# JuliaParallel/DistributedArrays.jl

Hardware: NVIDIA H100
Metric: GB/s for map! and sum on Float32 DArray (higher is better)
Workload: dtype f32

## Files before the change

### distributedarrays.jl_b200/_broadcast.py

```python
from __future__ import annotations

import ctypes as C
import struct
from typing import Callable, List, Optional, Sequence, Tuple

import numpy as np

from builtins import any as builtins_any

from . import _lib
from ._darray import B200Array, DArray, dab_dtype, darray, makelocal
from .layout import shape_of
from .runtime import runtime

_RANK = {"bool": 0, "i32": 1, "i64": 2, "i128": 3, "f32": 4, "f64": 5}


class _TagTypes(dict):

    def __missing__(self, tag):
        raise _lib.UnsupportedError(_lib.ERR_UNSUPPORTED, f"values of type {tag} have no array element type on the GPU backend "
                                    "(Int128 is served as the value type of mapreduce(f, op, d) only)")


# ... 407 lines not shown
        self.arr, self.scalar, self.tag, self.temp = arr, scalar, tag, temp


def run_local(rt, expr: Expr, out: B200Array, largs: List[LocalArg]):
    n = out.size
    if n == 0:
        return
    out_tag = tag_of(out.dtype)
    full = [a for a in largs if a.arr is not None]
    same = all(a.arr.shape == out.shape or a.arr.size == n and _squeeze(a.arr.shape) == _squeeze(out.shape) for a in full)
    ctx = rt.ctx
    code = dab_dtype(out.dtype)
    rt.last_kernel = "fixed"
    if same and expr.jt == out_tag and out_tag != "bool":
        x0 = largs[0] if largs and largs[0].arr is not None and largs[0].tag == out_tag else None
        if x0 is not None and all(_only_arg0(expr)):
            ab = match_affine(expr)
            if ab is not None:
                a = np.asarray(ab[0], dtype=out.dtype)
                b = np.asarray(ab[1], dtype=out.dtype)
                _lib.call("dab_affine", ctx, code, C.c_void_p(out.ptr), C.c_void_p(x0.arr.ptr), C.c_void_p(a.ctypes.data),
                          C.c_void_p(b.ctypes.data), n)
                rt.last_kernel = "dab_affine"
                return
            if expr.op in _UN and _is_arg(expr.args[0], 0):
                _lib.call("dab_unary", ctx, code, _UN[expr.op], C.c_void_p(out.ptr), C.c_void_p(x0.arr.ptr), n)
                return
            if _is_arg(expr, 0):
                _lib.call("dab_unary", ctx, code, _lib.MAP_ID, C.c_void_p(out.ptr), C.c_void_p(x0.arr.ptr), n)
                return
        if expr.op in _BIN and len(expr.args) == 2 and not (expr.op == "div" and out_tag[0] != "f"):
            l, r = expr.args
            la = largs[l.val] if l.op == "arg" else None
            ra = largs[r.val] if r.op == "arg" else None

            def arr_ok(e, a):
                return e.op == "arg" and a is not None and a.arr is not None and a.tag == out_tag

            def sc_val(e, a):
# ... 284 lines not shown
```

### distributedarrays.jl_b200/_darray.py

```python
from __future__ import annotations

import ctypes as C
import itertools
import weakref
from typing import Callable, Dict, List, Optional, Sequence, Tuple

import numpy as np

from . import _lib
from .layout import Layout, Range, default_procs, layout_from_chunk_shapes, make_layout, rlen, shape_of, slab_plan
from .runtime import Runtime, runtime

_DT = {np.dtype(np.float32): _lib.F32, np.dtype(np.float64): _lib.F64, np.dtype(np.int32): _lib.I32,
       np.dtype(np.int64): _lib.I64, np.dtype(np.bool_): _lib.U8}
_NP = {_lib.F32: np.dtype(np.float32), _lib.F64: np.dtype(np.float64), _lib.I32: np.dtype(np.int32),
       _lib.I64: np.dtype(np.int64), _lib.U8: np.dtype(np.bool_)}


def dab_dtype(dt) -> int:
    dt = np.dtype(dt)
    if dt not in _DT:
        raise _lib.UnsupportedError(_lib.ERR_UNSUPPORTED, f"element type {dt} is not served by the GPU backend (no host fallback)")
    return _DT[dt]

# ... 22 lines not shown
        dtype = np.dtype(dtype)
        n = int(np.prod(shape)) if len(shape) else 1
        ptr = rt.alloc_temp(n * dtype.itemsize) if temp else rt.alloc(n * dtype.itemsize)
        return cls(rt, ptr, shape, dtype, temp=temp)

    @classmethod
    def from_numpy(cls, rt: Runtime, a: np.ndarray) -> "B200Array":
        a = np.asarray(a)
        dab_dtype(a.dtype)
        out = cls.empty(rt, a.shape, a.dtype)
        out.copy_from_host(a)
        return out

    @property
    def size(self) -> int:
        return int(np.prod(self.shape)) if len(self.shape) else 1

    @property
    def nbytes(self) -> int:
        return self.size * self.dtype.itemsize

    @property
    def ndim(self) -> int:
        return len(self.shape)

    def copy_from_host(self, a: np.ndarray, sync: bool = True):
        a = np.asarray(a, dtype=self.dtype)
        if tuple(a.shape) != self.shape:
            raise _lib.DimensionMismatch(_lib.ERR_DIM_MISMATCH, f"host array {a.shape} vs chunk {self.shape}")
        if self.size == 0:
            return
# ... 657 lines not shown
```

### distributedarrays.jl_b200/_lib.py

```python
from __future__ import annotations

import ctypes as C
import os

_HERE = os.path.dirname(os.path.abspath(__file__))
SO_PATH = os.path.join(_HERE, "csrc", "libdab200.so")

OK, ERR_CUDA, ERR_ARG, ERR_EMPTY, ERR_DIM_MISMATCH, ERR_NCCL, ERR_UNSUPPORTED, ERR_NVRTC, ERR_NOMEM = range(9)
F32, F64, I32, I64, U8, I128 = range(6)
SUM, PROD, MAX, MIN, ALL, ANY, COUNT, EXTREMA = range(8)
MAP_ID, MAP_ABS, MAP_ABS2, MAP_NEG, MAP_SQRT, MAP_INV, MAP_FLOOR, MAP_CEIL, MAP_SIGN = range(9)
MAP_EQ, MAP_NE, MAP_LT, MAP_LE, MAP_GT, MAP_GE, MAP_ISNAN, MAP_NONZERO = range(16, 24)
ADD, SUB, MUL, DIV, REM, BMAX, BMIN, MOD, IDIV, AND, OR, XOR = range(12)
SORT_SLICES_SMEM_LEN = 8192
SVDVALS_MAX_K, SVDVALS_MAX_ELEMS = 32, 4096


class DabError(RuntimeError):

    def __init__(self, status: int, msg: str):
        super().__init__(f"[dab status {status}] {msg}")
        self.status = status


# ... 16 lines not shown
_pvp = C.POINTER(C.c_void_p)
_SZ4 = C.c_size_t * 4

_SIGS = {
    "dab_abi_version": (_i32, []),
    "dab_device_count": (_i32, [C.POINTER(_i32)]),
    "dab_init": (_i32, [_i32, _pvp]),
    "dab_shutdown": (_i32, [_vp]),
    "dab_last_error": (C.c_char_p, [_vp]),
    "dab_status_string": (C.c_char_p, [_i32]),
    "dab_sync": (_i32, [_vp]),
    "dab_device_info": (_i32, [_vp, C.POINTER(_i32), C.POINTER(_i32), C.POINTER(_sz), C.POINTER(_sz)]),
    "dab_stream": (_i32, [_vp, _pvp]),
    "dab_set_option": (_i32, [_vp, C.c_char_p, C.c_int64]),
    "dab_launch_count": (_i32, [_vp, C.POINTER(_u64)]),
    "dab_event_create": (_i32, [_vp, _pvp]),
    "dab_event_record": (_i32, [_vp, _vp]),
    "dab_event_elapsed_ms": (_i32, [_vp, _vp, _vp, C.POINTER(C.c_float)]),
    "dab_event_destroy": (_i32, [_vp, _vp]),
    "dab_alloc": (_i32, [_vp, _sz, _pvp]),
    "dab_free": (_i32, [_vp, _vp]),
    "dab_alloc_async": (_i32, [_vp, _sz, _pvp]),
    "dab_free_async": (_i32, [_vp, _vp]),
    "dab_host_alloc": (_i32, [_vp, _sz, _pvp]),
    "dab_host_free": (_i32, [_vp, _vp]),
    "dab_h2d": (_i32, [_vp, _vp, _vp, _sz]),
    "dab_d2h": (_i32, [_vp, _vp, _vp, _sz]),
    "dab_d2d": (_i32, [_vp, _vp, _vp, _sz]),
    "dab_h2d_2d": (_i32, [_vp, _vp, _sz, _vp, _sz, _sz, _sz]),
    "dab_d2h_2d": (_i32, [_vp, _vp, _sz, _vp, _sz, _sz, _sz]),
# ... 90 lines not shown
```

### distributedarrays.jl_b200/_mapreduce.py

```python
from __future__ import annotations

import builtins
import ctypes as C
import operator
from typing import Callable, Dict, Optional, Sequence, Tuple

import numpy as np

from . import _lib
from ._broadcast import Expr, broadcast, tag_of, trace, _NPT
from ._darray import B200Array, DArray, dab_dtype, np_dtype
from .layout import Layout, collapse_for_region, ravel, shape_of, unravel

_OPS = {"+": _lib.SUM, "add": _lib.SUM, "sum": _lib.SUM, "*": _lib.PROD, "mul": _lib.PROD, "prod": _lib.PROD, "max": _lib.MAX,
        "min": _lib.MIN}
_OPF = {operator.add: _lib.SUM, operator.mul: _lib.PROD, builtins.max: _lib.MAX, builtins.min: _lib.MIN, np.add: _lib.SUM,
        np.multiply: _lib.PROD, np.maximum: _lib.MAX, np.minimum: _lib.MIN}


def _op_code(op) -> int:
    if isinstance(op, str) and op in _OPS:
        return _OPS[op]
    if op in _OPF:
        return _OPF[op]
# ... 29 lines not shown
                    return side.args[0], Expr("const", (), tag, c) if -2**31 <= c < 2**31 or tag == "i64" else (side, const)
            return side, const

        l, r = unpromote(l, r)
        r, l = unpromote(r, l)
        if l.op == "arg" and r.op == "const" and l.jt == tag:
            return _CMPMAP[e.op], np.asarray(r.val, dtype=np.dtype(dtype)), e
        if r.op == "arg" and l.op == "const" and r.jt == tag:
            return _CMPMAP[_FLIP[e.op]], np.asarray(l.val, dtype=np.dtype(dtype)), e
    if e.op == "isnan" and e.args[0].op == "arg":
        return _lib.MAP_ISNAN, None, e
    return None, None, e


def _result_dtype(dtype, op: int, mapc: int) -> np.dtype:
    out = C.c_int32()
    _lib.check(_lib.lib().dab_reduce_result_dtype(dab_dtype(dtype), op, mapc, C.byref(out)))
    return np.dtype(np.int64) if out.value == _lib.I64 else np_dtype(out.value)




def _gather_slots(d: DArray, launch: Callable[[int, B200Array, int], None]) -> np.ndarray:
    rt = d.rt
    wpr = rt.workers_per_rank
    slots = B200Array.empty(rt, (16 * wpr,), np.uint8, temp=True)
    try:
        for pid, ch in d.chunks.items():
            launch(pid, ch, slots.ptr + 16 * ((pid - 1) % wpr))
        if rt.world > 1:
# ... 543 lines not shown
```

### distributedarrays.jl_b200/csrc/dab_comm.cu

```cuda
#include <dlfcn.h>
#include <nccl.h>

#include "dab_common.cuh"
#include "dab_scalar_ops.cuh"

namespace {

struct NcclApi {
    void* handle = nullptr;
    ncclResult_t (*GetUniqueId)(ncclUniqueId*) = nullptr;
    ncclResult_t (*CommInitRank)(ncclComm_t*, int, ncclUniqueId, int) = nullptr;
    ncclResult_t (*CommDestroy)(ncclComm_t) = nullptr;
    ncclResult_t (*AllGather)(const void*, void*, size_t, ncclDataType_t, ncclComm_t, cudaStream_t) = nullptr;
    ncclResult_t (*AllReduce)(const void*, void*, size_t, ncclDataType_t, ncclRedOp_t, ncclComm_t, cudaStream_t) = nullptr;
    ncclResult_t (*Send)(const void*, size_t, ncclDataType_t, int, ncclComm_t, cudaStream_t) = nullptr;
    ncclResult_t (*Recv)(void*, size_t, ncclDataType_t, int, ncclComm_t, cudaStream_t) = nullptr;
    ncclResult_t (*GroupStart)() = nullptr;
    ncclResult_t (*GroupEnd)() = nullptr;
    const char* (*GetErrorString)(ncclResult_t) = nullptr;
    const char* (*GetLastError)(ncclComm_t) = nullptr;
    bool ok = false;
    char why[256] = "";
};

// ... 188 lines not shown
    DAB_NCCL(ctx, api.Recv(recv_dev, nbytes, ncclInt8, peer, (ncclComm_t)ctx->comm, ctx->stream));
    return DAB_OK;
}

int32_t dab_mapreduce_all(dab_ctx* ctx, int32_t dtype, int32_t op, int32_t map, const void* map_param, const void* x, size_t n,
                          void* out_host) {
    DAB_ENTER_NOFLUSH(ctx);
    int32_t rdt;
    if (!out_host || op == DAB_EXTREMA || dab_reduce_result_dtype(dtype, op, map, &rdt) != DAB_OK) {
        DAB_FLUSH(ctx);
        DAB_REQUIRE(ctx, out_host, DAB_ERR_ARG, "dab_mapreduce_all: null out");
        if (op == DAB_EXTREMA) return dab_fail(ctx, DAB_ERR_UNSUPPORTED, "dab_mapreduce_all: extrema combines through dab_reduce + dab_allgather");
        return dab_fail(ctx, DAB_ERR_ARG, "bad dtype/op");
    }
    if ((ctx->mbox_ranks > 1 || !ctx->comm || ctx->nranks == 1) && n > 0) {
        ctx->fuse_op = op;
        int32_t st = dab_reduce(ctx, dtype, op, map, map_param, x, n, ctx->result_slot);
        ctx->fuse_op = -1;
        if (st != DAB_OK) return st;
        DAB_CUDA(ctx, cudaStreamSynchronize(ctx->stream));
        const volatile unsigned long long* h = (const volatile unsigned long long*)ctx->host_slot;
        if (h[1] != 0) return dab_fail(ctx, DAB_ERR_NCCL, "fused combine timed out waiting for a peer's chunk result (did every rank call?)");
        unsigned long long bits = h[0];
        memset(out_host, 0, 8);
        memcpy(out_host, &bits, dab_dtype_size(rdt));
        return DAB_OK;
    }
    int32_t st = dab_reduce(ctx, dtype, op, map, map_param, x, n, ctx->result_slot);
    if (st != DAB_OK) return st;
    const int P = ctx->comm ? ctx->nranks : 1;
    const void* src = ctx->result_slot;
    if (P > 1) {
        NEED_COMM(ctx);
        DAB_NCCL(ctx, api.AllGather(ctx->result_slot, ctx->gather_slots, 16, ncclInt8, (ncclComm_t)ctx->comm, ctx->stream));
        ctx->launches++;
// ... 140 lines not shown
```

### distributedarrays.jl_b200/csrc/dab_common.cuh

```cuda
#pragma once
#include <cuda_runtime.h>

#include <cstdint>
#include <cstdio>
#include <cstring>

#include "../../include/dab200.h"

#define DAB_MAX_REDUCE_BLOCKS 262144
#define DAB_SLOT_BYTES 64
#define DAB_MAX_RANKS 64

struct dab_pending_affine {
    int active;
    int32_t dtype;
    void* y;
    const void* x;
    size_t n;
    unsigned char a[8], b[8];
};

struct dab_ctx {
    int device;
    int sm_count;
// ... 18 lines not shown
    struct dab_alloc_cache* cache;
    void* sort_dev;
    size_t sort_dev_bytes;
    void* stage[2];
    cudaEvent_t stage_ev[2];
    void* sort_host;
    unsigned long long sort_epoch;
    long long opt_combine_timeout_ms;
    long long opt_gemm_kc;
    int opt_gemm_rawhi;
    int opt_gemm_simt;
    int opt_gemv_phase;
    int opt_gemv_t_cols;
    int opt_gemv_t_waves;
    int opt_ew_tma;
    dab_pending_affine pending;
    int defer_off;
    char err[512];
};

extern thread_local char dab_tls_err[512];

int32_t dab_fail(dab_ctx* ctx, int32_t status, const char* fmt, ...);
int32_t dab_fail_cuda(dab_ctx* ctx, cudaError_t e, const char* what, const char* file, int line);

#define DAB_CUDA(ctx, call)                                                             \
    do {                                                                                \
        cudaError_t e__ = (call);                                                       \
        if (e__ != cudaSuccess) return dab_fail_cuda((ctx), e__, #call, __FILE__, __LINE__); \
    } while (0)
// ... 19 lines not shown
        DAB_CUDA((ctx), cudaSetDevice((ctx)->device));                      \
        DAB_FLUSH(ctx);                                                     \
    } while (0)

#define DAB_ENTER_NOFLUSH(ctx)                                              \
    do {                                                                    \
        if ((ctx) == nullptr) return dab_fail(nullptr, DAB_ERR_ARG, "null ctx"); \
        DAB_CUDA((ctx), cudaSetDevice((ctx)->device));                      \
    } while (0)

#define DAB_LAUNCHED(ctx)                          \
    do {                                           \
        (ctx)->launches++;                         \
        DAB_CUDA((ctx), cudaGetLastError());       \
    } while (0)

static inline size_t dab_dtype_size(int32_t dt) {
    switch (dt) {
        case DAB_F32: return 4;
        case DAB_F64: return 8;
        case DAB_I32: return 4;
        case DAB_I64: return 8;
        case DAB_U8: return 1;
        default: return 0;
    }
}

#define DAB_MBOX_SLOT 32
#define DAB_MBOX_BARRIER_OFFSET (2 * DAB_MAX_RANKS * DAB_MBOX_SLOT)
#define DAB_MBOX_BYTES (DAB_MBOX_BARRIER_OFFSET + DAB_MAX_RANKS * 8)
// ... 56 lines not shown
```

### distributedarrays.jl_b200/csrc/dab_core.cu

```cuda
#include <cstdarg>
#include <cstdlib>
#include <map>
#include <mutex>
#include <new>
#include <thread>
#include <unordered_map>

#include "dab_common.cuh"

thread_local char dab_tls_err[512] = "";

struct dab_alloc_cache {
    std::unordered_map<void*, size_t> live;
    std::multimap<size_t, void*> free_blocks;
    size_t cached_bytes = 0;
    static constexpr size_t kMaxBlock = 16ull << 30;
    static constexpr size_t kMaxCached = 32ull << 30;
};

int dab_resident_ctas(const void* kernel, int threads) {
    static std::mutex mu;
    static std::unordered_map<const void*, int> cache;
    std::lock_guard<std::mutex> lk(mu);
    auto it = cache.find(kernel);
// ... 60 lines not shown
    if (!out) return dab_fail(nullptr, DAB_ERR_ARG, "null ctx out-pointer");
    *out = nullptr;
    int n = 0;
    cudaError_t e = cudaGetDeviceCount(&n);
    if (e != cudaSuccess) return dab_fail_cuda(nullptr, e, "cudaGetDeviceCount", __FILE__, __LINE__);
    if (device < 0 || device >= n) return dab_fail(nullptr, DAB_ERR_ARG, "device %d out of range (have %d)", device, n);
    dab_ctx* ctx = new (std::nothrow) dab_ctx();
    if (!ctx) return dab_fail(nullptr, DAB_ERR_NOMEM, "host allocation failed");
    memset(ctx, 0, sizeof(*ctx));
    ctx->device = device;
    ctx->rank = 0;
    ctx->nranks = 1;
    ctx->fuse_op = -1;
    ctx->opt_combine_timeout_ms = 120000;
    ctx->opt_gemv_phase = 1;
    ctx->opt_gemv_t_waves = 4;
    ctx->opt_gemv_t_cols = 8;
    ctx->cache = new (std::nothrow) dab_alloc_cache();
#define INIT_CUDA(call)                                                     \
    do {                                                                    \
        cudaError_t e__ = (call);                                           \
        if (e__ != cudaSuccess) {                                           \
            int32_t st = dab_fail_cuda(nullptr, e__, #call, __FILE__, __LINE__); \
            delete ctx;                                                     \
            return st;                                                      \
        }                                                                   \
    } while (0)
    INIT_CUDA(cudaSetDevice(device));
    cudaDeviceProp prop;
    INIT_CUDA(cudaGetDeviceProperties(&prop, device));
// ... 3 lines not shown
                        prop.major, prop.minor);
    }
    ctx->sm_count = prop.multiProcessorCount;
    INIT_CUDA(cudaStreamCreateWithFlags(&ctx->stream, cudaStreamNonBlocking));
    {
        cudaMemPool_t pool;
        INIT_CUDA(cudaDeviceGetDefaultMemPool(&pool, device));
        unsigned long long keep = ~0ull;
        INIT_CUDA(cudaMemPoolSetAttribute(pool, cudaMemPoolAttrReleaseThreshold, &keep));
    }
    INIT_CUDA(cudaMalloc(&ctx->block_partials, ((size_t)DAB_MAX_REDUCE_BLOCKS + DAB_MAX_REDUCE_BLOCKS / 256 + 16) * 16));
    INIT_CUDA(cudaMalloc((void**)&ctx->counter, (DAB_MAX_REDUCE_BLOCKS / 256 + 16) * 4));
    INIT_CUDA(cudaMemsetAsync(ctx->counter, 0, (DAB_MAX_REDUCE_BLOCKS / 256 + 16) * 4, ctx->stream));
    INIT_CUDA(cudaMalloc(&ctx->result_slot, DAB_SLOT_BYTES));
    INIT_CUDA(cudaMalloc(&ctx->gather_slots, (size_t)DAB_MAX_RANKS * 16));
    INIT_CUDA(cudaHostAlloc(&ctx->host_slot, (size_t)(DAB_MAX_RANKS + 2) * 16, cudaHostAllocDefault));
    INIT_CUDA(cudaStreamSynchronize(ctx->stream));
    memset(ctx->host_slot, 0, (size_t)(DAB_MAX_RANKS + 2) * 16);
#undef INIT_CUDA
    *out = ctx;
    return DAB_OK;
}

int32_t dab_comm_destroy(dab_ctx* ctx);
int32_t dab_mailbox_detach(dab_ctx* ctx);

int32_t dab_shutdown(dab_ctx* ctx) {
    if (!ctx) return DAB_OK;
    cudaSetDevice(ctx->device);
    const int32_t st = dab_flush_pending(ctx);
    cudaStreamSynchronize(ctx->stream);
    if (ctx->comm) dab_comm_destroy(ctx);
    cudaFree(ctx->block_partials);
// ... 48 lines not shown
    ctx->defer_off = 1;
    *stream = (void*)ctx->stream;
    return DAB_OK;
}

int32_t dab_set_option(dab_ctx* ctx, const char* key, int64_t value) {
    if (!ctx || !key) return dab_fail(ctx, DAB_ERR_ARG, "null argument");
    if (ctx->pending.active) {
        DAB_CUDA(ctx, cudaSetDevice(ctx->device));
        DAB_FLUSH(ctx);
    }
    if (strcmp(key, "ew_tma") == 0) {
        ctx->opt_ew_tma = value != 0;
        return DAB_OK;
    }
    if (strcmp(key, "gemm_kc") == 0) {
        ctx->opt_gemm_kc = value;
        return DAB_OK;
    }
    if (strcmp(key, "gemm_rawhi") == 0) {
        ctx->opt_gemm_rawhi = value != 0;
        return DAB_OK;
    }
    if (strcmp(key, "gemv_phase") == 0) {
        ctx->opt_gemv_phase = value != 0;
        return DAB_OK;
    }
    if (strcmp(key, "gemv_t_cols") == 0) {
        if (value != 4 && value != 8) return dab_fail(ctx, DAB_ERR_ARG, "gemv_t_cols must be 4 or 8");
        ctx->opt_gemv_t_cols = (int)value;
// ... 11 lines not shown
    if (strcmp(key, "combine_timeout_ms") == 0) {
        if (value < 1) return dab_fail(ctx, DAB_ERR_ARG, "combine_timeout_ms must be >= 1");
        ctx->opt_combine_timeout_ms = value;
        return DAB_OK;
    }
    return dab_fail(ctx, DAB_ERR_ARG, "dab_set_option: unknown key %s", key);
}

int32_t dab_launch_count(dab_ctx* ctx, uint64_t* launches) {
    if (!ctx || !launches) return dab_fail(ctx, DAB_ERR_ARG, "null argument");
    if (ctx->pending.active) {
        DAB_CUDA(ctx, cudaSetDevice(ctx->device));
        DAB_FLUSH(ctx);
    }
    *launches = ctx->launches;
    return DAB_OK;
}

int32_t dab_event_create(dab_ctx* ctx, void** event) {
    DAB_ENTER(ctx);
    DAB_REQUIRE(ctx, event, DAB_ERR_ARG, "null event out-pointer");
    cudaEvent_t ev;
    DAB_CUDA(ctx, cudaEventCreate(&ev));
    *event = (void*)ev;
    return DAB_OK;
}
int32_t dab_event_record(dab_ctx* ctx, void* event) {
    DAB_ENTER(ctx);
    DAB_CUDA(ctx, cudaEventRecord((cudaEvent_t)event, ctx->stream));
    return DAB_OK;
// ... 249 lines not shown
```

### distributedarrays.jl_b200/csrc/dab_reduce.cu

```cuda
#include <type_traits>

#include <cmath>

#include "dab_reduce_traits.cuh"

namespace {

constexpr int RD_UNROLL = 4;

struct NoStore {
    template <typename T>
    __device__ __forceinline__ void vec(Pack<T>&, size_t) const {}
    template <typename T>
    __device__ __forceinline__ T scalar(T v, size_t) const { return v; }
};
template <typename T>
struct AffineStore {
    AffineF<T> f;
    T* y;
    int4* yv;
    __device__ __forceinline__ void vec(Pack<T>& p, size_t i) const {
#pragma unroll
        for (int k = 0; k < Pack<T>::N; ++k) p.v[k] = f(p.v[k]);
        st_stream(yv + i, as_int4(p));
    }
    __device__ __forceinline__ T scalar(T v, size_t i) const {
        v = f(v);
        y[i] = v;
        return v;
    }
};

template <typename T, typename Map, typename R, typename Out, typename St>
__global__ void __launch_bounds__(RD_THREADS, 8) reduce_kernel(const T* __restrict__ x, size_t n, size_t head, Map map,
                                                             typename R::A* __restrict__ partials, unsigned int* counter,
                                                             void* out, int finalize_mode, long long n_for_all, int tiles_per_cta,
                                                             FusedComm fc, St st) {
    using A = typename R::A;
    using V = typename Map::V;
    constexpr int VPT = 16 / sizeof(T);
    __shared__ A smem[RD_THREADS / 32];
    __shared__ bool is_last;

    const size_t nvec = (n - head) / VPT;
    const int4* xv = reinterpret_cast<const int4*>(x + head);
    constexpr size_t TILE = (size_t)RD_THREADS * RD_UNROLL;
    const size_t ntiles = nvec / TILE;
    A acc = R::identity();
    size_t t_end = ((size_t)blockIdx.x + 1) * (size_t)tiles_per_cta;
    if (t_end > ntiles) t_end = ntiles;
#pragma unroll 1
    for (size_t t = (size_t)blockIdx.x * (size_t)tiles_per_cta; t < t_end; ++t) {
        const size_t base = t * TILE + threadIdx.x;
        int4 r[RD_UNROLL];
#pragma unroll
        for (int u = 0; u < RD_UNROLL; ++u) r[u] = ld_stream(xv + base + (size_t)u * RD_THREADS);
        V tv[RD_UNROLL];
#pragma unroll
        for (int u = 0; u < RD_UNROLL; ++u) {
            Pack<T> p = as_pack<T>(r[u]);
            st.vec(p, base + (size_t)u * RD_THREADS);
            V m[VPT];
#pragma unroll
            for (int k = 0; k < VPT; ++k) m[k] = map(p.v[k]);
#pragma unroll
            for (int w = VPT; w > 1; w >>= 1)
#pragma unroll
                for (int k = 0; k < w / 2; ++k) m[k] = R::tile(m[k], m[k + w / 2]);
            tv[u] = m[0];
        }
#pragma unroll
        for (int w = RD_UNROLL; w > 1; w >>= 1)
#pragma unroll
            for (int k = 0; k < w / 2; ++k) tv[k] = R::tile(tv[k], tv[k + w / 2]);
        acc = R::comb(acc, R::lift(tv[0]));
    }
    if (blockIdx.x == gridDim.x - 1) {
        for (size_t i = ntiles * TILE + threadIdx.x; i < nvec; i += RD_THREADS) {
            Pack<T> p = as_pack<T>(ld_stream(xv + i));
            st.vec(p, i);
            V m = map(p.v[0]);
#pragma unroll
            for (int k = 1; k < VPT; ++k) m = R::tile(m, map(p.v[k]));
            acc = R::comb(acc, R::lift(m));
        }
        for (size_t i = threadIdx.x; i < head; i += RD_THREADS) acc = R::comb(acc, R::lift(map(st.scalar(x[i], i))));
        for (size_t i = head + nvec * VPT + threadIdx.x; i < n; i += RD_THREADS) acc = R::comb(acc, R::lift(map(st.scalar(x[i], i))));
    }
    acc = block_reduce<R>(acc, smem);
    A* gpartials = partials + DAB_MAX_REDUCE_BLOCKS;
// ... 39 lines not shown
            if (fc.host_out && fc.nranks <= 1) {
                unsigned long long bits = 0;
                memcpy(&bits, &res, sizeof(Out));
                volatile unsigned long long* h = reinterpret_cast<volatile unsigned long long*>(fc.host_out);
                h[0] = bits;
                h[1] = 0ull;
                __threadfence_system();
            }
        } else {
            memset(out, 0, 16);
            memcpy(out, &fin, sizeof(A));
        }
    }
    if constexpr (!std::is_arithmetic<Out>::value) return;
    else {
    if (fc.nranks <= 1) return;
    __shared__ unsigned long long pay[2];
    __shared__ unsigned long long got[DAB_MAX_RANKS];
    __shared__ int timed_out;
    if (threadIdx.x == 0) {
        memcpy(&pay[0], out, 8);
        memcpy(&pay[1], (char*)out + 8, 8);
        timed_out = 0;
    }
    __syncthreads();
    const size_t bank = (size_t)(fc.seq & 1ull) * DAB_MAX_RANKS * DAB_MBOX_SLOT;
    if (threadIdx.x < (unsigned)fc.nranks) {
        volatile unsigned long long* dst =
            reinterpret_cast<volatile unsigned long long*>((char*)fc.peers[threadIdx.x] + bank + (size_t)fc.rank * DAB_MBOX_SLOT);
        dst[0] = pay[0];
        dst[1] = pay[1];
// ... 22 lines not shown
            switch (fc.op) {
                case DAB_SUM: case DAB_COUNT: a = jl::add(a, b); break;
                case DAB_PROD: a = jl::mul(a, b); break;
                case DAB_MAX: a = jl::max(a, b); break;
                case DAB_MIN: a = jl::min(a, b); break;
                case DAB_ALL: a = (Out)(a != (Out)0 && b != (Out)0); break;
                default: a = (Out)(a != (Out)0 || b != (Out)0); break;
            }
        }
        unsigned long long bits = 0;
        memcpy(&bits, &a, sizeof(Out));
        volatile unsigned long long* h = reinterpret_cast<volatile unsigned long long*>(fc.host_out);
        h[0] = bits;
        h[1] = (unsigned long long)timed_out;
        __threadfence_system();
    }
    }
}

template <typename T, typename Map, typename R, typename Out, typename St = NoStore>
int32_t launch_reduce(dab_ctx* ctx, const T* x, size_t n, Map map, void* out, int finalize_mode, St st = St()) {
    constexpr int VPT = 16 / sizeof(T);
    size_t head = ((16 - ((uintptr_t)x & 15)) & 15) / sizeof(T);
    if (head > n) head = n;
    if constexpr (!std::is_same<St, NoStore>::value) st.yv = reinterpret_cast<int4*>(st.y + head);
    size_t tiles = (n - head) / ((size_t)VPT * RD_THREADS * RD_UNROLL);
    size_t k = 2;
    if ((tiles + k - 1) / k > (size_t)DAB_MAX_REDUCE_BLOCKS) k = (tiles + DAB_MAX_REDUCE_BLOCKS - 1) / DAB_MAX_REDUCE_BLOCKS;
    size_t grid = (tiles + k - 1) / k;
    if (grid < 1) grid = 1;
// ... 60 lines not shown
#define P(FN) \
    case FN: return reduce_pred<T, FN>(ctx, op, x, n, param, out)
            P(DAB_MAP_EQ);
            P(DAB_MAP_NE);
            P(DAB_MAP_LT);
            P(DAB_MAP_LE);
            P(DAB_MAP_GT);
            P(DAB_MAP_GE);
            P(DAB_MAP_ISNAN);
            P(DAB_MAP_NONZERO);
#undef P
        default: return dab_fail(ctx, DAB_ERR_UNSUPPORTED, "map %d not served by a reduce kernel (no host fallback)", map);
    }
}

template <typename T>
int32_t reduce_pending_affine(dab_ctx* ctx, int32_t op, const dab_pending_affine& p, void* out) {
    using M = MapF<T, DAB_MAP_ID>;
    AffineStore<T> st;
    memcpy(&st.f.a, p.a, sizeof(T));
    memcpy(&st.f.b, p.b, sizeof(T));
    st.y = (T*)p.y;
    st.yv = nullptr;
    const T* x = (const T*)p.x;
    switch (op) {
        case DAB_SUM: return launch_reduce<T, M, SumTraits<T>, ResultOfSum<T>>(ctx, x, p.n, M{(T)0}, out, 0, st);
        case DAB_PROD: return launch_reduce<T, M, ProdTraits<T>, ResultOfSum<T>>(ctx, x, p.n, M{(T)0}, out, 0, st);
        case DAB_MAX: return launch_reduce<T, M, MaxTraits<T>, T>(ctx, x, p.n, M{(T)0}, out, 0, st);
        default: return launch_reduce<T, M, MinTraits<T>, T>(ctx, x, p.n, M{(T)0}, out, 0, st);
    }
}

bool consumes_pending(const dab_ctx* ctx, int32_t dtype, int32_t op, int32_t map, const void* x, size_t n) {
    const dab_pending_affine& p = ctx->pending;
    return p.active && x == p.y && n == p.n && dtype == p.dtype && map == DAB_MAP_ID &&
           (op == DAB_SUM || op == DAB_PROD || op == DAB_MAX || op == DAB_MIN);
}

// ... 58 lines not shown
        case DAB_MIN:
        case DAB_EXTREMA: *out_dtype = dtype; return DAB_OK;
        case DAB_ALL:
        case DAB_ANY:
        case DAB_COUNT: *out_dtype = DAB_I64; return DAB_OK;
        default: return DAB_ERR_ARG;
    }
}

int32_t dab_reduce(dab_ctx* ctx, int32_t dtype, int32_t op, int32_t map, const void* map_param, const void* x, size_t n,
                   void* out_dev) {
    DAB_ENTER_NOFLUSH(ctx);
    if (out_dev && consumes_pending(ctx, dtype, op, map, x, n)) {
        const dab_pending_affine p = ctx->pending;
        ctx->pending.active = 0;
        switch (dtype) {
            case DAB_F32: return reduce_pending_affine<float>(ctx, op, p, out_dev);
            case DAB_F64: return reduce_pending_affine<double>(ctx, op, p, out_dev);
            case DAB_I32: return reduce_pending_affine<int32_t>(ctx, op, p, out_dev);
            default: return reduce_pending_affine<long long>(ctx, op, p, out_dev);
        }
    }
    DAB_FLUSH(ctx);
    DAB_REQUIRE(ctx, out_dev && (x || n == 0), DAB_ERR_ARG, "dab_reduce: null pointer");
    DAB_REQUIRE(ctx, op >= DAB_SUM && op <= DAB_EXTREMA, DAB_ERR_ARG, "dab_reduce: bad op %d", op);
    if (n == 0) return empty_result(ctx, dtype, op, out_dev);
    switch (dtype) {
        case DAB_F32: return reduce_t<float>(ctx, op, map, map_param, (const float*)x, n, out_dev);
        case DAB_F64: return reduce_t<double>(ctx, op, map, map_param, (const double*)x, n, out_dev);
        case DAB_I32: return reduce_t<int32_t>(ctx, op, map, map_param, (const int32_t*)x, n, out_dev);
        case DAB_I64: return reduce_t<long long>(ctx, op, map, map_param, (const long long*)x, n, out_dev);
        case DAB_U8: return reduce_u8(ctx, op, map, (const uint8_t*)x, n, out_dev);
        default: return dab_fail(ctx, DAB_ERR_ARG, "dab_reduce: bad dtype %d", dtype);
    }
}
// ... 107 lines not shown
```

### distributedarrays.jl_b200/runtime.py

```python
from __future__ import annotations

import ctypes as C
import os
from typing import List, Optional

import numpy as np

from . import _lib

_RT: Optional["Runtime"] = None


class Runtime:
    def __init__(self, workers_per_rank: int = 1, device: Optional[int] = None, use_dist: Optional[bool] = None):
        L = _lib.lib()
        self.rank = int(os.environ.get("RANK", "0"))
        self.world = int(os.environ.get("WORLD_SIZE", "1"))
        self.local_rank = int(os.environ.get("LOCAL_RANK", "0"))
        self.workers_per_rank = int(workers_per_rank)
        n = C.c_int32(0)
        _lib.check(L.dab_device_count(C.byref(n)))
        if n.value < 1:
            raise _lib.DabError(_lib.ERR_CUDA, "no CUDA device visible: the DArray hot path has no CPU fallback")
        self.device = int(device) if device is not None else self.local_rank % n.value
# ... 147 lines not shown
        _lib.call("dab_alloc_async", self.ctx, int(nbytes), C.byref(p))
        return int(p.value)

    def free_temp(self, ptr: int):
        if ptr and self.ctx:
            _lib.call("dab_free_async", self.ctx, C.c_void_p(ptr))

    def set_option(self, key: str, value: int):
        _lib.call("dab_set_option", self.ctx, key.encode(), int(value))

    def launches(self) -> int:
        n = C.c_uint64(0)
        _lib.call("dab_launch_count", self.ctx, C.byref(n))
        return int(n.value)

    def device_info(self):
        dev, sms, fr, tot = C.c_int32(), C.c_int32(), C.c_size_t(), C.c_size_t()
        _lib.call("dab_device_info", self.ctx, C.byref(dev), C.byref(sms), C.byref(fr), C.byref(tot))
        return {"device": dev.value, "sm_count": sms.value, "free_bytes": fr.value, "total_bytes": tot.value}

    def event(self) -> int:
        e = C.c_void_p()
        _lib.call("dab_event_create", self.ctx, C.byref(e))
        return int(e.value)

    def record(self, ev: int):
        _lib.call("dab_event_record", self.ctx, C.c_void_p(ev))

    def elapsed_ms(self, e0: int, e1: int) -> float:
        ms = C.c_float()
# ... 75 lines not shown
```

### include/dab200.h

```cpp
#ifndef DAB200_H
#define DAB200_H

#include <stddef.h>
#include <stdint.h>

#ifdef __cplusplus
extern "C" {
#endif

#define DAB_ABI_VERSION 1

typedef struct dab_ctx dab_ctx;

enum {
    DAB_OK = 0,
    DAB_ERR_CUDA = 1,
    DAB_ERR_ARG = 2,
    DAB_ERR_EMPTY = 3,
    DAB_ERR_DIM_MISMATCH = 4,
    DAB_ERR_NCCL = 5,
    DAB_ERR_UNSUPPORTED = 6,
    DAB_ERR_NVRTC = 7,
    DAB_ERR_NOMEM = 8
};
// ... 34 lines not shown
    DAB_IDIV = 8 ,
    DAB_AND = 9, DAB_OR = 10, DAB_XOR = 11
};

int32_t dab_abi_version(void);
int32_t dab_device_count(int32_t* count);
int32_t dab_init(int32_t device, dab_ctx** ctx);
int32_t dab_shutdown(dab_ctx* ctx);
const char* dab_last_error(const dab_ctx* ctx);
const char* dab_status_string(int32_t status);
int32_t dab_sync(dab_ctx* ctx);
int32_t dab_device_info(dab_ctx* ctx, int32_t* device, int32_t* sm_count, size_t* free_bytes, size_t* total_bytes);
int32_t dab_stream(dab_ctx* ctx, void** stream);
int32_t dab_set_option(dab_ctx* ctx, const char* key, int64_t value);
int32_t dab_launch_count(dab_ctx* ctx, uint64_t* launches);

int32_t dab_event_create(dab_ctx* ctx, void** event);
int32_t dab_event_record(dab_ctx* ctx, void* event);
int32_t dab_event_elapsed_ms(dab_ctx* ctx, void* start, void* stop, float* ms);
int32_t dab_event_destroy(dab_ctx* ctx, void* event);

int32_t dab_alloc(dab_ctx* ctx, size_t nbytes, void** dptr);
int32_t dab_free(dab_ctx* ctx, void* dptr);
int32_t dab_alloc_async(dab_ctx* ctx, size_t nbytes, void** dptr);
int32_t dab_free_async(dab_ctx* ctx, void* dptr);
int32_t dab_host_alloc(dab_ctx* ctx, size_t nbytes, void** hptr);
int32_t dab_host_free(dab_ctx* ctx, void* hptr);
int32_t dab_h2d(dab_ctx* ctx, void* dptr, const void* hptr, size_t nbytes);
int32_t dab_d2h(dab_ctx* ctx, void* hptr, const void* dptr, size_t nbytes);
int32_t dab_d2d(dab_ctx* ctx, void* dst, const void* src, size_t nbytes);
// ... 93 lines not shown
```

Measured before the change: 4338.

## Prefetch next tile in fused affine-reduce kernel and trim Python dispatch overhead

Adds a software-pipelined path to the fused map!+sum reduce kernel that loads the next tile into registers while folding the current one, with launch bounds relaxed to 4 blocks per SM to leave room for the extra registers. This path is on by default through a new fused_prefetch option. It also moves the affine match ahead of the arg0-only check, caches result-dtype lookups, and uses math.prod for sizes to cut host overhead. Optional globaltimer/host step timestamps are added for profiling; they add a pointer check to the kernel and cost fewer resident blocks when the prefetch path is taken.

Result: faster. 4429 (median of 6 runs) (+2.1%).

```diff
diff --git a/distributedarrays.jl_b200/_broadcast.py b/distributedarrays.jl_b200/_broadcast.py
--- a/distributedarrays.jl_b200/_broadcast.py
+++ b/distributedarrays.jl_b200/_broadcast.py
@@ -445,15 +445,15 @@
     rt.last_kernel = "fixed"
     if same and expr.jt == out_tag and out_tag != "bool":
         x0 = largs[0] if largs and largs[0].arr is not None and largs[0].tag == out_tag else None
+        ab = match_affine(expr) if x0 is not None else None
+        if ab is not None:
+            a = np.asarray(ab[0], dtype=out.dtype)
+            b = np.asarray(ab[1], dtype=out.dtype)
+            _lib.call("dab_affine", ctx, code, C.c_void_p(out.ptr), C.c_void_p(x0.arr.ptr), C.c_void_p(a.ctypes.data),
+                      C.c_void_p(b.ctypes.data), n)
+            rt.last_kernel = "dab_affine"
+            return
         if x0 is not None and all(_only_arg0(expr)):
-            ab = match_affine(expr)
-            if ab is not None:
-                a = np.asarray(ab[0], dtype=out.dtype)
-                b = np.asarray(ab[1], dtype=out.dtype)
-                _lib.call("dab_affine", ctx, code, C.c_void_p(out.ptr), C.c_void_p(x0.arr.ptr), C.c_void_p(a.ctypes.data),
-                          C.c_void_p(b.ctypes.data), n)
-                rt.last_kernel = "dab_affine"
-                return
             if expr.op in _UN and _is_arg(expr.args[0], 0):
                 _lib.call("dab_unary", ctx, code, _UN[expr.op], C.c_void_p(out.ptr), C.c_void_p(x0.arr.ptr), n)
                 return
diff --git a/distributedarrays.jl_b200/_darray.py b/distributedarrays.jl_b200/_darray.py
--- a/distributedarrays.jl_b200/_darray.py
+++ b/distributedarrays.jl_b200/_darray.py
@@ -2,6 +2,7 @@
 
 import ctypes as C
 import itertools
+import math
 import weakref
 from typing import Callable, Dict, List, Optional, Sequence, Tuple
 
@@ -60,7 +61,7 @@
 
     @property
     def size(self) -> int:
-        return int(np.prod(self.shape)) if len(self.shape) else 1
+        return int(math.prod(self.shape))
 
     @property
     def nbytes(self) -> int:
diff --git a/distributedarrays.jl_b200/_lib.py b/distributedarrays.jl_b200/_lib.py
--- a/distributedarrays.jl_b200/_lib.py
+++ b/distributedarrays.jl_b200/_lib.py
@@ -54,6 +54,7 @@
     "dab_stream": (_i32, [_vp, _pvp]),
     "dab_set_option": (_i32, [_vp, C.c_char_p, C.c_int64]),
     "dab_launch_count": (_i32, [_vp, C.POINTER(_u64)]),
+    "dab_step_timestamps": (_i32, [_vp, C.POINTER(_u64)]),
     "dab_event_create": (_i32, [_vp, _pvp]),
     "dab_event_record": (_i32, [_vp, _vp]),
     "dab_event_elapsed_ms": (_i32, [_vp, _vp, _vp, C.POINTER(C.c_float)]),
diff --git a/distributedarrays.jl_b200/_mapreduce.py b/distributedarrays.jl_b200/_mapreduce.py
--- a/distributedarrays.jl_b200/_mapreduce.py
+++ b/distributedarrays.jl_b200/_mapreduce.py
@@ -2,6 +2,7 @@
 
 import builtins
 import ctypes as C
+import functools
 import operator
 from typing import Callable, Dict, Optional, Sequence, Tuple
 
@@ -67,6 +68,11 @@
 
 
 def _result_dtype(dtype, op: int, mapc: int) -> np.dtype:
+    return _result_dtype_of(np.dtype(dtype), op, mapc)
+
+
+@functools.lru_cache(maxsize=None)
+def _result_dtype_of(dtype: np.dtype, op: int, mapc: int) -> np.dtype:
     out = C.c_int32()
     _lib.check(_lib.lib().dab_reduce_result_dtype(dab_dtype(dtype), op, mapc, C.byref(out)))
     return np.dtype(np.int64) if out.value == _lib.I64 else np_dtype(out.value)
diff --git a/distributedarrays.jl_b200/csrc/dab_comm.cu b/distributedarrays.jl_b200/csrc/dab_comm.cu
--- a/distributedarrays.jl_b200/csrc/dab_comm.cu
+++ b/distributedarrays.jl_b200/csrc/dab_comm.cu
@@ -1,10 +1,17 @@
 #include <dlfcn.h>
 #include <nccl.h>
+#include <time.h>
 
 #include "dab_common.cuh"
 #include "dab_scalar_ops.cuh"
 
 namespace {
+
+uint64_t monotonic_ns() {
+    timespec t;
+    clock_gettime(CLOCK_MONOTONIC, &t);
+    return (uint64_t)t.tv_sec * 1000000000ull + (uint64_t)t.tv_nsec;
+}
 
 struct NcclApi {
     void* handle = nullptr;
@@ -226,11 +233,15 @@
         return dab_fail(ctx, DAB_ERR_ARG, "bad dtype/op");
     }
     if ((ctx->mbox_ranks > 1 || !ctx->comm || ctx->nranks == 1) && n > 0) {
+        const bool stamp = ctx->opt_step_timestamps != 0;
+        if (stamp) ctx->step_host_ns[0] = monotonic_ns();
         ctx->fuse_op = op;
         int32_t st = dab_reduce(ctx, dtype, op, map, map_param, x, n, ctx->result_slot);
         ctx->fuse_op = -1;
         if (st != DAB_OK) return st;
+        if (stamp) ctx->step_host_ns[1] = monotonic_ns();
         DAB_CUDA(ctx, cudaStreamSynchronize(ctx->stream));
+        if (stamp) ctx->step_host_ns[2] = monotonic_ns();
         const volatile unsigned long long* h = (const volatile unsigned long long*)ctx->host_slot;
         if (h[1] != 0) return dab_fail(ctx, DAB_ERR_NCCL, "fused combine timed out waiting for a peer's chunk result (did every rank call?)");
         unsigned long long bits = h[0];
diff --git a/distributedarrays.jl_b200/csrc/dab_common.cuh b/distributedarrays.jl_b200/csrc/dab_common.cuh
--- a/distributedarrays.jl_b200/csrc/dab_common.cuh
+++ b/distributedarrays.jl_b200/csrc/dab_common.cuh
@@ -56,6 +56,9 @@
     int opt_gemv_t_cols;
     int opt_gemv_t_waves;
     int opt_ew_tma;
+    int opt_fused_prefetch;
+    int opt_step_timestamps;
+    uint64_t step_host_ns[3];
     dab_pending_affine pending;
     int defer_off;
     char err[512];
@@ -105,6 +108,11 @@
         (ctx)->launches++;                         \
         DAB_CUDA((ctx), cudaGetLastError());       \
     } while (0)
+
+#define DAB_HOST_SLOT_BYTES ((size_t)(DAB_MAX_RANKS + 3) * 16)
+static inline volatile unsigned long long* dab_step_stamps(dab_ctx* ctx) {
+    return (volatile unsigned long long*)((char*)ctx->host_slot + (DAB_MAX_RANKS + 2) * 16);
+}
 
 static inline size_t dab_dtype_size(int32_t dt) {
     switch (dt) {
diff --git a/distributedarrays.jl_b200/csrc/dab_core.cu b/distributedarrays.jl_b200/csrc/dab_core.cu
--- a/distributedarrays.jl_b200/csrc/dab_core.cu
+++ b/distributedarrays.jl_b200/csrc/dab_core.cu
@@ -98,6 +98,7 @@
     ctx->fuse_op = -1;
     ctx->opt_combine_timeout_ms = 120000;
     ctx->opt_gemv_phase = 1;
+    ctx->opt_fused_prefetch = 1;
     ctx->opt_gemv_t_waves = 4;
     ctx->opt_gemv_t_cols = 8;
     ctx->cache = new (std::nothrow) dab_alloc_cache();
@@ -131,9 +132,9 @@
     INIT_CUDA(cudaMemsetAsync(ctx->counter, 0, (DAB_MAX_REDUCE_BLOCKS / 256 + 16) * 4, ctx->stream));
     INIT_CUDA(cudaMalloc(&ctx->result_slot, DAB_SLOT_BYTES));
     INIT_CUDA(cudaMalloc(&ctx->gather_slots, (size_t)DAB_MAX_RANKS * 16));
-    INIT_CUDA(cudaHostAlloc(&ctx->host_slot, (size_t)(DAB_MAX_RANKS + 2) * 16, cudaHostAllocDefault));
+    INIT_CUDA(cudaHostAlloc(&ctx->host_slot, DAB_HOST_SLOT_BYTES, cudaHostAllocDefault));
     INIT_CUDA(cudaStreamSynchronize(ctx->stream));
-    memset(ctx->host_slot, 0, (size_t)(DAB_MAX_RANKS + 2) * 16);
+    memset(ctx->host_slot, 0, DAB_HOST_SLOT_BYTES);
 #undef INIT_CUDA
     *out = ctx;
     return DAB_OK;
@@ -212,6 +213,14 @@
         ctx->opt_ew_tma = value != 0;
         return DAB_OK;
     }
+    if (strcmp(key, "fused_prefetch") == 0) {
+        ctx->opt_fused_prefetch = value != 0;
+        return DAB_OK;
+    }
+    if (strcmp(key, "step_timestamps") == 0) {
+        ctx->opt_step_timestamps = value != 0;
+        return DAB_OK;
+    }
     if (strcmp(key, "gemm_kc") == 0) {
         ctx->opt_gemm_kc = value;
         return DAB_OK;
@@ -253,6 +262,15 @@
         DAB_FLUSH(ctx);
     }
     *launches = ctx->launches;
+    return DAB_OK;
+}
+
+int32_t dab_step_timestamps(dab_ctx* ctx, uint64_t* out5) {
+    if (!ctx || !out5) return dab_fail(ctx, DAB_ERR_ARG, "null argument");
+    const volatile unsigned long long* d = dab_step_stamps(ctx);
+    out5[0] = d[0];
+    out5[1] = d[1];
+    for (int k = 0; k < 3; ++k) out5[2 + k] = ctx->step_host_ns[k];
     return DAB_OK;
 }
 
diff --git a/distributedarrays.jl_b200/csrc/dab_reduce.cu b/distributedarrays.jl_b200/csrc/dab_reduce.cu
--- a/distributedarrays.jl_b200/csrc/dab_reduce.cu
+++ b/distributedarrays.jl_b200/csrc/dab_reduce.cu
@@ -9,16 +9,21 @@
 constexpr int RD_UNROLL = 4;
 
 struct NoStore {
+    static constexpr int kMinBlocks = 8;
+    static constexpr bool kPrefetch = false;
     template <typename T>
     __device__ __forceinline__ void vec(Pack<T>&, size_t) const {}
     template <typename T>
     __device__ __forceinline__ T scalar(T v, size_t) const { return v; }
 };
-template <typename T>
+template <typename T, bool PF>
 struct AffineStore {
+    static constexpr int kMinBlocks = PF ? 4 : 8;
+    static constexpr bool kPrefetch = PF;
     AffineF<T> f;
     T* y;
     int4* yv;
+    volatile unsigned long long* ts;
     __device__ __forceinline__ void vec(Pack<T>& p, size_t i) const {
 #pragma unroll
         for (int k = 0; k < Pack<T>::N; ++k) p.v[k] = f(p.v[k]);
@@ -31,8 +36,34 @@
     }
 };
 
+template <typename T, typename Map, typename R, typename St>
+__device__ __forceinline__ typename R::A fold_tile(typename R::A acc, const int4 (&r)[RD_UNROLL], size_t base, const Map& map,
+                                                   const St& st) {
+    using V = typename Map::V;
+    constexpr int VPT = 16 / sizeof(T);
+    V tv[RD_UNROLL];
+#pragma unroll
+    for (int u = 0; u < RD_UNROLL; ++u) {
+        Pack<T> p = as_pack<T>(r[u]);
+        st.vec(p, base + (size_t)u * RD_THREADS);
+        V m[VPT];
+#pragma unroll
+        for (int k = 0; k < VPT; ++k) m[k] = map(p.v[k]);
+#pragma unroll
+        for (int w = VPT; w > 1; w >>= 1)
+#pragma unroll
+            for (int k = 0; k < w / 2; ++k) m[k] = R::tile(m[k], m[k + w / 2]);
+        tv[u] = m[0];
+    }
+#pragma unroll
+    for (int w = RD_UNROLL; w > 1; w >>= 1)
+#pragma unroll
+        for (int k = 0; k < w / 2; ++k) tv[k] = R::tile(tv[k], tv[k + w / 2]);
+    return R::comb(acc, R::lift(tv[0]));
+}
+
 template <typename T, typename Map, typename R, typename Out, typename St>
-__global__ void __launch_bounds__(RD_THREADS, 8) reduce_kernel(const T* __restrict__ x, size_t n, size_t head, Map map,
+__global__ void __launch_bounds__(RD_THREADS, St::kMinBlocks) reduce_kernel(const T* __restrict__ x, size_t n, size_t head, Map map,
                                                              typename R::A* __restrict__ partials, unsigned int* counter,
                                                              void* out, int finalize_mode, long long n_for_all, int tiles_per_cta,
                                                              FusedComm fc, St st) {
@@ -42,6 +73,9 @@
     __shared__ A smem[RD_THREADS / 32];
     __shared__ bool is_last;
 
+    if constexpr (!std::is_same<St, NoStore>::value) {
+        if (st.ts && blockIdx.x == 0 && threadIdx.x == 0) st.ts[0] = dab_globaltimer_ns();
+    }
     const size_t nvec = (n - head) / VPT;
     const int4* xv = reinterpret_cast<const int4*>(x + head);
     constexpr size_t TILE = (size_t)RD_THREADS * RD_UNROLL;
@@ -49,6 +83,25 @@
     A acc = R::identity();
     size_t t_end = ((size_t)blockIdx.x + 1) * (size_t)tiles_per_cta;
     if (t_end > ntiles) t_end = ntiles;
+    if constexpr (St::kPrefetch) {
+        size_t t = (size_t)blockIdx.x * (size_t)tiles_per_cta;
+        int4 r[RD_UNROLL];
+        if (t < t_end) {
+#pragma unroll
+            for (int u = 0; u < RD_UNROLL; ++u) r[u] = ld_stream(xv + t * TILE + threadIdx.x + (size_t)u * RD_THREADS);
+        }
+#pragma unroll 1
+        for (; t < t_end; ++t) {
+            int4 nx[RD_UNROLL];
+            if (t + 1 < t_end) {
+#pragma unroll
+                for (int u = 0; u < RD_UNROLL; ++u) nx[u] = ld_stream(xv + (t + 1) * TILE + threadIdx.x + (size_t)u * RD_THREADS);
+            }
+            acc = fold_tile<T, Map, R>(acc, r, t * TILE + threadIdx.x, map, st);
+#pragma unroll
+            for (int u = 0; u < RD_UNROLL; ++u) r[u] = nx[u];
+        }
+    } else {
 #pragma unroll 1
     for (size_t t = (size_t)blockIdx.x * (size_t)tiles_per_cta; t < t_end; ++t) {
         const size_t base = t * TILE + threadIdx.x;
@@ -74,6 +127,7 @@
 #pragma unroll
             for (int k = 0; k < w / 2; ++k) tv[k] = R::tile(tv[k], tv[k + w / 2]);
         acc = R::comb(acc, R::lift(tv[0]));
+    }
     }
     if (blockIdx.x == gridDim.x - 1) {
         for (size_t i = ntiles * TILE + threadIdx.x; i < nvec; i += RD_THREADS) {
@@ -143,7 +197,12 @@
     }
     if constexpr (!std::is_arithmetic<Out>::value) return;
     else {
-    if (fc.nranks <= 1) return;
+    if (fc.nranks <= 1) {
+        if constexpr (!std::is_same<St, NoStore>::value) {
+            if (st.ts && threadIdx.x == 0) st.ts[1] = dab_globaltimer_ns();
+        }
+        return;
+    }
     __shared__ unsigned long long pay[2];
     __shared__ unsigned long long got[DAB_MAX_RANKS];
     __shared__ int timed_out;
@@ -196,6 +255,9 @@
         h[0] = bits;
         h[1] = (unsigned long long)timed_out;
         __threadfence_system();
+        if constexpr (!std::is_same<St, NoStore>::value) {
+            if (st.ts) st.ts[1] = dab_globaltimer_ns();
+        }
     }
     }
 }
@@ -286,14 +348,15 @@
     }
 }
 
-template <typename T>
+template <typename T, bool PF>
 int32_t reduce_pending_affine(dab_ctx* ctx, int32_t op, const dab_pending_affine& p, void* out) {
     using M = MapF<T, DAB_MAP_ID>;
-    AffineStore<T> st;
+    AffineStore<T, PF> st;
     memcpy(&st.f.a, p.a, sizeof(T));
     memcpy(&st.f.b, p.b, sizeof(T));
     st.y = (T*)p.y;
     st.yv = nullptr;
+    st.ts = ctx->opt_step_timestamps ? dab_step_stamps(ctx) : nullptr;
     const T* x = (const T*)p.x;
     switch (op) {
         case DAB_SUM: return launch_reduce<T, M, SumTraits<T>, ResultOfSum<T>>(ctx, x, p.n, M{(T)0}, out, 0, st);
@@ -382,11 +445,19 @@
     if (out_dev && consumes_pending(ctx, dtype, op, map, x, n)) {
         const dab_pending_affine p = ctx->pending;
         ctx->pending.active = 0;
+        if (ctx->opt_fused_prefetch) {
+            switch (dtype) {
+                case DAB_F32: return reduce_pending_affine<float, true>(ctx, op, p, out_dev);
+                case DAB_F64: return reduce_pending_affine<double, true>(ctx, op, p, out_dev);
+                case DAB_I32: return reduce_pending_affine<int32_t, true>(ctx, op, p, out_dev);
+                default: return reduce_pending_affine<long long, true>(ctx, op, p, out_dev);
+            }
+        }
         switch (dtype) {
-            case DAB_F32: return reduce_pending_affine<float>(ctx, op, p, out_dev);
-            case DAB_F64: return reduce_pending_affine<double>(ctx, op, p, out_dev);
-            case DAB_I32: return reduce_pending_affine<int32_t>(ctx, op, p, out_dev);
-            default: return reduce_pending_affine<long long>(ctx, op, p, out_dev);
+            case DAB_F32: return reduce_pending_affine<float, false>(ctx, op, p, out_dev);
+            case DAB_F64: return reduce_pending_affine<double, false>(ctx, op, p, out_dev);
+            case DAB_I32: return reduce_pending_affine<int32_t, false>(ctx, op, p, out_dev);
+            default: return reduce_pending_affine<long long, false>(ctx, op, p, out_dev);
         }
     }
     DAB_FLUSH(ctx);
diff --git a/distributedarrays.jl_b200/runtime.py b/distributedarrays.jl_b200/runtime.py
--- a/distributedarrays.jl_b200/runtime.py
+++ b/distributedarrays.jl_b200/runtime.py
@@ -2,7 +2,7 @@
 
 import ctypes as C
 import os
-from typing import List, Optional
+from typing import List, Optional, Tuple
 
 import numpy as np
 
@@ -185,6 +185,11 @@
         _lib.call("dab_launch_count", self.ctx, C.byref(n))
         return int(n.value)
 
+    def step_timestamps(self) -> Tuple[int, ...]:
+        buf = (C.c_uint64 * 5)()
+        _lib.call("dab_step_timestamps", self.ctx, buf)
+        return tuple(int(v) for v in buf)
+
     def device_info(self):
         dev, sms, fr, tot = C.c_int32(), C.c_int32(), C.c_size_t(), C.c_size_t()
         _lib.call("dab_device_info", self.ctx, C.byref(dev), C.byref(sms), C.byref(fr), C.byref(tot))
diff --git a/include/dab200.h b/include/dab200.h
--- a/include/dab200.h
+++ b/include/dab200.h
@@ -72,6 +72,7 @@
 int32_t dab_stream(dab_ctx* ctx, void** stream);
 int32_t dab_set_option(dab_ctx* ctx, const char* key, int64_t value);
 int32_t dab_launch_count(dab_ctx* ctx, uint64_t* launches);
+int32_t dab_step_timestamps(dab_ctx* ctx, uint64_t* out5);
 
 int32_t dab_event_create(dab_ctx* ctx, void** event);
 int32_t dab_event_record(dab_ctx* ctx, void* event);
```
